# petitioner/MOAI-FHE-TransformerInference-Public

Measured on AMD Instinct MI355X. Metric: NTT+INTT algorithmic GB/s (N=2^16, L=44x60-bit, batch=256 ciphertexts/GPU) vs HBM peak, higher is better.
Workload: dtype u64; 1 GPU; configs[1]: negacyclic NTT then INTT, N=65536, 44 x 60-bit primes, 256 ciphertexts x 2 polys per GPU; batch_per_gpu=256, batch_total=256, coeff_modulus=CoeffModulus::Create(65536, 44 x 60), bytes_per_coeff_per_transform=16

## Files before the change

### moai-fhe-transformerinference-public_amd/csrc/launch.h

```cpp
#pragma once
#include <type_traits>

#include "common.h"
#include "rowlaunch.h"

namespace moai {

#define MOAI_KNOBS(X)                                                                                                          \
    X(NTT_FP, 1, "0: primes below 2^51 stay on the integer units in every transform, key switch and mod-down")                \
    X(NTT_LAZY8, 1, "0: integer primes below 2^60 take the exact butterflies instead of the approximate Shoup quotient")       \
    X(NTT_LAZY16, 1, "0: those primes keep values below 8q with a guard in every stage instead of below 16q with fewer (M_LAZY8)") \
    X(NTT_LDSTW, 1, "0: the forward contiguous pass loads its first stages' twiddles from memory instead of through LDS")      \
    X(NTT_CHUNK_MB, 88, "> 0: launch the two passes of a transform per chunk of whole polynomials of at most this many MiB")    \
    X(NTT_CHUNK_KB, 0, "KiB added to MOAI_NTT_CHUNK_MB: chunks of rings whose polynomials are smaller than a MiB")             \
    X(NTT_PIPE, 2, "1..3: deal those chunks to this many side streams, so that a chunk's second pass runs beside the next one's first; 0: one stream") \
    X(NTT_PIPE_MIN, 32, "chunks per side stream below which a transform stays on the caller's stream")                         \
    X(NTT_PIPE_INNER, 0, "1: the transforms inside key switch, mod-down, encode and decode take the MOAI_NTT_PIPE schedule too") \
    X(NTT_NAIVE, 0, "1: one launch per radix-2 stage over global memory (cross-check path)")                                   \
    X(KS_FP_MIN_ROWS, 16, "batch * L from which the key switch uses the FP64 arithmetic modes")                                \
    X(KS_TMP_MB, 8192, "MiB of key-switch digits in flight: sets how many output moduli share a launch")                       \
    X(KS_P1_ITEMS, 8, "1: the key switch's strided pass at N = 2^16 runs one tile per workgroup instead of eight, pipelined")  \
    X(KS_HOIST_PAIR, 4, "rotations per pass of the hoisted MAC in the FP64 modes: 4, 2, or 0 for one")                         \
    X(MD_FP_MIN_ROWS, 256, "polynomials * L from which mod-down and rescale use the FP64 arithmetic modes")                    \
    X(MATMUL_FP, 1, "0: moai_ct_pt_matmul keeps primes below 2^51 on the integer kernel")                                      \
    X(DEC_TMP_MB, 1024, "MiB of scratch per chunk of moai_ckks_decode when the stream's arena is smaller")                     \
    X(CLIENT_TMP_KB, 1048576, "KiB of scratch per chunk of the encryption and key generation calls when the stream's arena is smaller") \
    X(HYBRID_TMP_KB, 16777216, "KiB of scratch per chunk of the hybrid key switch: sets how many ciphertexts of a batch are in flight") \
    X(HYBRID_HOIST_NR, 4, "rotations per pass of the hybrid hoisted MAC over the digits: 4, 2 or 1")

enum Knob
{
#define MOAI_KNOB_ID(id, dflt, what) K_##id,
    MOAI_KNOBS(MOAI_KNOB_ID)
#undef MOAI_KNOB_ID
    KNOB_COUNT
};
long tuning(Knob k);

template <int... Vs, class F>
int dispatch(const char *what, int v, F &&f)
{
    int rc = MOAI_OK;
    const bool found = ((v == Vs && ((rc = f(std::integral_constant<int, Vs>{})), true)) || ...);
    return found ? rc : set_error(MOAI_ELOGIC, "unsupported %s%d", what, v);
}
template <class F>
int dispatch_logn(int logn, F &&f)
{
    return dispatch<12, 13, 14, 15, 16>("poly_modulus_degree 2^", logn, f);
}
template <class F>
int for_chunks(size_t n, size_t per, F &&f)
{
    for (size_t x0 = 0; x0 < n; x0 += per)
    {
        MOAI_TRY(f(x0, n - x0 < per ? n - x0 : per));
    }
    return MOAI_OK;
}
template <class F>
int for_term_chunks(size_t terms, size_t per, F &&f)
{
    return terms ? for_chunks(terms, per, f) : f(0, 0);
}
inline bool overlap(const void *a, size_t a_bytes, const void *b, size_t b_bytes)
{
    const uintptr_t x = (uintptr_t)a, y = (uintptr_t)b;
    return x < y + b_bytes && y < x + a_bytes;
}
void trace_op(const char *name, size_t L, size_t units);
bool noguard_ok(uint64_t q);
int enter_device(const moai_ctx *c);
int ntt_mode(const moai_ctx *c, uint32_t prime, bool allow_fp = true);
int fwd_class(const moai_ctx *c, uint32_t prime);
int inv_class(const moai_ctx *c, uint32_t prime);
struct TwPair
{
    const Tw *tw, *twb;
};
TwPair twiddles(const moai_ctx *c, int mode, bool inverse);
struct NttArgs;
NttArgs ntt_args(const moai_ctx *c, uint64_t *data, size_t n_poly, size_t L, const RowMap &rows, bool inverse);
int make_rowmap(const moai_ctx *c, size_t L, const uint32_t *prime_index, RowMap *out);
int rows_entry(const moai_ctx *c, size_t L, const uint32_t *prime_index, RowMap *out);
int ntt_launch(moai_ctx *c, uint64_t *data, size_t n_poly, size_t L, const RowMap &rows, bool inverse,
               hipStream_t s, const uint64_t *src = nullptr, size_t src_stride_rows = 0, size_t src_off_rows = 0, bool entry = false);
size_t ntt_pipe_plan(size_t n_poly, size_t L, size_t n, size_t chunk_bytes, long k, long min_chunks, size_t *chunk_polys = nullptr,
                     int *streams = nullptr);
moai_ctx::NttPipe *ntt_pipe(moai_ctx *c, hipStream_t s);
int workspace(moai_ctx *c, size_t bytes, hipStream_t s, void **out);
size_t chunk_items(moai_ctx *c, hipStream_t s, size_t per_bytes, size_t n, size_t cap, size_t floor_bytes);
int reserve_for_stream(moai_ctx *c, void *stream, size_t bytes, void **out, bool headroom);
int galois_table(moai_ctx *c, uint32_t elt, const uint32_t **out);
int galois_permute_c0(moai_ctx *c, const uint64_t *in, uint64_t *out, size_t batch, size_t L, uint32_t galois_elt, hipStream_t s);
int galois_sign_mask(moai_ctx *c, uint64_t *mask, uint32_t galois_elt, size_t copies, hipStream_t s);
int probe_any_zero(moai_ctx *c, const uint64_t *v, size_t words, uint32_t *flag, hipStream_t s, bool *found);
int galois_elt_check(const moai_ctx *c, uint32_t elt);
int moddown_finalize(moai_ctx *c, const uint64_t *acc, uint32_t acc_stride, const uint64_t *u, uint64_t *out, size_t P, size_t Lout,
                     const Tw *inv, const KsAddend &add, const KsList *lst, hipStream_t s);
int galois_gather_list(moai_ctx *c, const KsList *lst, uint64_t *out, size_t members, size_t rows_per_member, size_t src_off_rows,
                       hipStream_t s);
int ks_list_write(const KsList &h, KsList *d, hipStream_t s);
int ks_list_check_members(const uint64_t *const *ins, uint64_t *const *outs, const uint32_t *elts, const uint64_t *const *keys,
                          const uint64_t *one_key, size_t n, bool relin);
int ks_list_check_blocks(const moai_ctx *c, const uint64_t *const *ins, uint64_t *const *outs, const uint32_t *elts,
                         const uint64_t *const *sums, size_t n, size_t in_bytes, size_t out_bytes, bool relin);

int ensure_ckks_tables(moai_ctx *c);
int total_coeff_bits(const moai_ctx *c, size_t L, const uint32_t *prime_index);

size_t rescale_ws_bytes(const moai_ctx *c, size_t L, size_t polys);
int rescale_nolock(moai_ctx *c, const uint64_t *in, uint64_t *out, size_t size, size_t L, size_t batch, hipStream_t s);

int encrypt_zero_key_level(moai_ctx *c, const uint8_t *key, uint64_t seq, const uint64_t *sk_ntt, uint64_t *out, size_t n_batch,
                           hipStream_t s);

int seal_uniform_launch(moai_ctx *c, const uint8_t *seeds, uint64_t *out, size_t stride_words, size_t count, size_t L,
                        const RowMap &rows, uint32_t *cnt, uint32_t *rejected, hipStream_t s);

}
```

### moai-fhe-transformerinference-public_amd/csrc/ntt.hip

```cpp
#include <mutex>

#include "ntt_kernels.hip.h"
#include "launch.h"

namespace moai {

bool noguard_ok(uint64_t q)
{
    return q < (~0ull) / 36;
}

int ntt_mode(const moai_ctx *c, uint32_t prime, bool allow_fp)
{
    const int m = (int)c->pc_host[prime].fp_mode;
    if (allow_fp && m && tuning(K_NTT_FP))
    {
        return m;
    }
    return noguard_ok(c->primes[prime]) ? M_NOGUARD : M_GUARD;
}

TwPair twiddles(const moai_ctx *c, int mode, bool inverse)
{
    if (mode_fp(mode))
    {
        return inverse ? TwPair{ c->inv_twf, c->inv_twfb } : TwPair{ c->fwd_twf, c->fwd_twfb };
    }
    return inverse ? TwPair{ c->inv_tw, c->inv_twb } : TwPair{ c->fwd_tw, c->fwd_twb };
}

static bool lazy8_ok(const moai_ctx *c, uint32_t prime)
{
    return tuning(K_NTT_LAZY8) && c->primes[prime] < (1ull << 60);
}
static bool lazy16_ok(const moai_ctx *c, uint32_t prime)
{
    return lazy8_ok(c, prime) && tuning(K_NTT_LAZY16);
}

int fwd_class(const moai_ctx *c, uint32_t prime)
{
    const int m = ntt_mode(c, prime);
    if (m != M_GUARD)
    {
        return m;
    }
    return lazy16_ok(c, prime) ? M_LAZY16 : (lazy8_ok(c, prime) ? M_LAZY8 : M_GUARD2);
}

int inv_class(const moai_ctx *c, uint32_t prime)
{
    const int m = ntt_mode(c, prime);
    if (mode_fp(m))
    {
        return m;
    }
    return lazy16_ok(c, prime) ? M_LAZY16 : (lazy8_ok(c, prime) ? M_LAZY8 : M_GUARD);
}

NttArgs ntt_args(const moai_ctx *c, uint64_t *data, size_t n_poly, size_t L, const RowMap &rows, bool inverse)
{
    NttArgs a;
    const TwPair t = twiddles(c, M_GUARD, inverse);
    a.data = data;
    a.tw = t.tw;
    a.twb = t.twb;
    a.pc = c->pc;
    a.rows = rows;
    for (size_t r = 0; r < MOAI_MAX_RNS; ++r)
    {
        a.sel.idx[r] = (uint32_t)(r < L ? r : 0);
        a.selp.idx[r] = rows.idx[r < L ? r : 0];
    }
    a.Lsel = (uint32_t)L;
    a.L = (uint32_t)L;
    a.n_poly = (uint32_t)n_poly;
    a.total_work = 0;
    a.src = nullptr;
    a.src_stride = a.src_off = 0;
    a.lds_twiddles = tuning(K_NTT_LDSTW) ? 1u : 0u;
    return a;
}

template <int LOGN, int MODE>
static void launch_fwd_mode(const NttArgs &a, hipStream_t s)
{
    hipLaunchKernelGGL((ntt_fwd_strided<LOGN, MODE>), dim3(a.total_work), dim3(256), 0, s, a);
    if constexpr (MODE == M_LAZY16)
    {
        if (a.lds_twiddles)
        {
            hipLaunchKernelGGL((ntt_fwd_contig<LOGN, MODE, 1>), dim3(a.total_work), dim3(256), 0, s, a);
        }
        else
        {
            hipLaunchKernelGGL((ntt_fwd_contig<LOGN, MODE, 0>), dim3(a.total_work), dim3(256), 0, s, a);
        }
    }
    else
    {
        hipLaunchKernelGGL((ntt_fwd_contig<LOGN, MODE>), dim3(a.total_work), dim3(256), 0, s, a);
    }
}

static void select_class(const moai_ctx *c, int (*row_class)(const moai_ctx *, uint32_t), int mode, NttArgs &a)
{
    a.Lsel = 0;
    for (uint32_t r = 0; r < a.L; ++r)
    {
        const uint32_t prime = a.rows.idx[r];
        if (row_class(c, prime) == mode)
        {
            a.selp.idx[a.Lsel] = prime;
            a.sel.idx[a.Lsel++] = r;
        }
    }
}

template <int LOGN, bool INV, int... MODES>
static int launch_classes(const moai_ctx *c, const NttArgs &base, hipStream_t s)
{
    for (int mode : { MODES... })
    {
        NttArgs a = base;
        select_class(c, INV ? inv_class : fwd_class, mode, a);
        if (a.Lsel == 0)
        {
            continue;
        }
        const TwPair t = twiddles(c, mode, INV);
        a.tw = t.tw;
        a.twb = t.twb;
        a.total_work = a.n_poly * a.Lsel * (1u << (LOGN - 12));
        MOAI_TRY((dispatch<MODES...>(INV ? "inverse transform mode " : "forward transform mode ", mode, [&](auto MD) {
            constexpr int MODE = decltype(MD)::value;
            if constexpr (INV)
            {
                hipLaunchKernelGGL((ntt_inv_contig<LOGN, MODE>), dim3(a.total_work), dim3(256), 0, s, a);
                hipLaunchKernelGGL((ntt_inv_strided<LOGN, MODE>), dim3(a.total_work), dim3(256), 0, s, a);
            }
            else
            {
                launch_fwd_mode<LOGN, MODE>(a, s);
            }
            return MOAI_OK;
        })));
    }
    return MOAI_OK;
}

template <int LOGN>
static int launch_fwd(const moai_ctx *c, const NttArgs &base, hipStream_t s)
{
    return launch_classes<LOGN, false, M_LAZY16, M_LAZY8, M_GUARD2, M_NOGUARD, M_FPN, M_FPR>(c, base, s);
}

template <int LOGN>
static int launch_inv(const moai_ctx *c, const NttArgs &base, hipStream_t s)
{
    return launch_classes<LOGN, true, M_GUARD, M_LAZY8, M_FPN, M_FPR, M_LAZY16>(c, base, s);
}

size_t ntt_pipe_plan(size_t n_poly, size_t L, size_t n, size_t chunk_bytes, long k, long min_chunks, size_t *chunk_polys, int *streams)
{
    size_t chunk = n_poly, per_stream = 0;
    int nk = 0;
    if (n_poly && L && n && chunk_bytes)
    {
        const size_t poly_bytes = L > (~(size_t)0) / sizeof(uint64_t) / n ? ~(size_t)0 : L * n * sizeof(uint64_t);
        chunk = chunk_bytes / poly_bytes;
        chunk = chunk < 1 ? 1 : (chunk > n_poly ? n_poly : chunk);
    }
    const size_t chunks = chunk ? (n_poly + chunk - 1) / chunk : 0;
    if (k >= 1 && chunks >= 2)
    {
        nk = k > NTT_PIPE_MAX ? NTT_PIPE_MAX : (int)k;
        nk = (size_t)nk > chunks ? (int)chunks : nk;
        per_stream = (chunks + (size_t)nk - 1) / (size_t)nk;
        if (min_chunks > 0 && per_stream < (size_t)min_chunks)
        {
            nk = 0;
            per_stream = 0;
        }
    }
    if (chunk_polys)
    {
        *chunk_polys = chunk;
    }
    if (streams)
    {
        *streams = nk;
    }
    return per_stream;
}

int ntt_launch(moai_ctx *c, uint64_t *data, size_t n_poly, size_t L, const RowMap &rows, bool inverse, hipStream_t s,
               const uint64_t *src, size_t src_stride_rows, size_t src_off_rows, bool entry)
{
    if (n_poly == 0 || L == 0)
    {
        return MOAI_OK;
    }
    if (src && !inverse)
    {
        return set_error(MOAI_ELOGIC, "only the inverse transform reads from another buffer");
    }
    if (src && (src_stride_rows > 0xffffffffull || src_off_rows > 0xffffffffull || src_off_rows + L > src_stride_rows))
    {
        return set_error(MOAI_EINVAL, "source slice outside its layout");
    }
    if (n_poly * L * (c->n >> (c->logn >= 12 ? 12 : 0)) > 0x7fffffffull || n_poly > 0xffffffffull)
    {
        return set_error(MOAI_EINVAL, "batch too large for one launch");
    }
    NttArgs a = ntt_args(c, data, n_poly, L, rows, inverse);
    const int logn = c->logn;
    const bool naive = tuning(K_NTT_NAIVE) != 0;
    if (src)
    {
        if (naive || logn <= 11)
        {
            const size_t row_bytes = c->n * sizeof(uint64_t);
            MOAI_HIP_CHECK(hipMemcpy2DAsync(data, L * row_bytes, src + src_off_rows * c->n, src_stride_rows * row_bytes, L * row_bytes, n_poly,
                                            hipMemcpyDeviceToDevice, s));
        }
        else
        {
            a.src = src;
            a.src_stride = (uint32_t)src_stride_rows;
            a.src_off = (uint32_t)src_off_rows;
        }
    }
    if (naive && logn >= 1)
    {
        const dim3 grid = row_grid(c, n_poly * L);
        if (!inverse)
        {
            for (int st = 0; st < logn; ++st)
            {
                hipLaunchKernelGGL(ntt_stage_global<false>, grid, dim3(256), 0, s, a, logn, st, st == logn - 1);
            }
        }
        else
        {
            for (int st = logn - 1; st >= 0; --st)
            {
                hipLaunchKernelGGL(ntt_stage_global<true>, grid, dim3(256), 0, s, a, logn, st, st == 0);
            }
        }
        MOAI_LAUNCH_CHECK();
        return MOAI_OK;
    }
    if (logn <= 11)
    {
        dim3 grid((uint32_t)(n_poly * L));
        if (inverse)
        {
            hipLaunchKernelGGL(ntt_small<true>, grid, dim3(256), 0, s, a, logn);
        }
        else
        {
            hipLaunchKernelGGL(ntt_small<false>, grid, dim3(256), 0, s, a, logn);
        }
        MOAI_LAUNCH_CHECK();
        return MOAI_OK;
    }
    size_t chunk = n_poly;
    int nk = 0;
    const long chunk_mb = tuning(K_NTT_CHUNK_MB), chunk_kb = tuning(K_NTT_CHUNK_KB);
    const size_t chunk_bytes = ((size_t)(chunk_mb > 0 ? chunk_mb : 0) << 20) + ((size_t)(chunk_kb > 0 ? chunk_kb : 0) << 10);
    const long want = tuning(K_NTT_PIPE);
    ntt_pipe_plan(n_poly, L, c->n, chunk_bytes, want > 0 && (entry || tuning(K_NTT_PIPE_INNER)) ? want : 0, tuning(K_NTT_PIPE_MIN), &chunk,
                  &nk);
    moai_ctx::NttPipe *pipe = nullptr;
    if (nk > 0)
    {
        hipStreamCaptureStatus cap = hipStreamCaptureStatusNone;
        if (hipStreamIsCapturing(s, &cap) != hipSuccess)
        {
            (void)hipGetLastError();
        }
        else if (cap == hipStreamCaptureStatusNone)
        {
            pipe = ntt_pipe(c, s);
        }
    }
    std::unique_lock<std::mutex> pipe_lock;
    if (want > 0 && !pipe)
    {
        chunk = n_poly;
    }
    if (pipe)
    {
        pipe_lock = std::unique_lock<std::mutex>(*static_cast<std::mutex *>(pipe->mu));
        MOAI_HIP_CHECK(hipEventRecord(pipe->fork, s));
        for (int i = 0; i < nk; ++i)
// ... 112 lines not shown
```

### moai-fhe-transformerinference-public_amd/csrc/ntt_kernels.hip.h

```cpp
#pragma once
#include "modarith.hip.h"

namespace moai {

__device__ __forceinline__ uint32_t xcd_remap(uint32_t b, uint32_t total)
{
    if (total & 7u)
    {
        return b;
    }
    return (b & 7u) * (total >> 3) + (b >> 3);
}

__device__ __forceinline__ void lds_barrier()
{
    asm volatile("s_waitcnt lgkmcnt(0)\n\ts_barrier" ::: "memory");
}

__device__ __forceinline__ void lds_wave_sync()
{
    asm volatile("s_waitcnt lgkmcnt(0)" ::: "memory");
}

__device__ __forceinline__ uint32_t phys_contig(uint32_t e)
// ... 341 lines not shown
    const uint32_t blk = (tile << 4) + b;
    const Tw *__restrict__ twbt = twb + (size_t)tile * (15 * 256);

    const bool use_lds = TWL < 0 ? ldstw != nullptr : TWL == 1;
    Tw fill;
    uint32_t fill_slot = 0;
    if (use_lds)
    {
        const uint32_t lane = tid & 63u;
        if (TWL == 1)
        {
            const uint32_t l = lane < 59u ? lane : 59u;
            const uint32_t bb = ((tid >> 6) << 2) + l / 15u, i = l % 15u;
            const uint32_t u = i == 0 ? 0u : (i < 3 ? 1u : (i < 7 ? 2u : 3u)), k = i - ((1u << u) - 1u);
            fill = tw[(1u << (R1 + u)) + (((tile << 4) + bb) << u) + k];
            fill_slot = bb * 15u + i;
        }
        else if (lane < 60u)
        {
            const uint32_t bb = ((tid >> 6) << 2) + lane / 15u, i = lane % 15u;
            const uint32_t u = i == 0 ? 0u : (i < 3 ? 1u : (i < 7 ? 2u : 3u)), k = i - ((1u << u) - 1u);
            ldstw[bb * 15u + i] = tw[(1u << (R1 + u)) + (((tile << 4) + bb) << u) + k];
        }
    }
    uint64_t x[16];
#pragma unroll
    for (int j = 0; j < 16; ++j)
    {
        x[j] = base[(b << 8) | ((uint32_t)j << 4) | tl];
    }
    if (use_lds)
    {
        if (TWL == 1 && (tid & 63u) < 60u)
        {
            ldstw[fill_slot] = fill;
        }
        lds_wave_sync();
    }
#pragma unroll
    for (int u = 0; u < 4; ++u)
    {
        const int half = 8 >> u;
#pragma unroll
        for (int j = 0; j < 16; ++j)
        {
            if (!(j & half))
            {
                Tw t = use_lds ? ldstw[b * 15u + ((1u << u) - 1u) + (uint32_t)(j >> (4 - u))]
                               : tw[(1u << (R1 + u)) + (blk << u) + (uint32_t)(j >> (4 - u))];
                ct_bfly_stage<MODE, LOGN>(x[j], x[j + half], t.w, t.wq, q, q2, 7 - u);
            }
        }
    }
#pragma unroll
    for (int j = 0; j < 16; ++j)
    {
        lds[phys_contig((b << 8) | ((uint32_t)j << 4) | tl)] = x[j];
    }
    lds_wave_sync();
    const uint32_t myrow = tid;
#pragma unroll
    for (int c = 0; c < 8; ++c)
    {
        ulonglong2 v = lds2[(myrow << 3) | ((uint32_t)c ^ (myrow & 7u))];
        x[2 * c] = v.x;
        x[2 * c + 1] = v.y;
    }
#pragma unroll
    for (int u = 4; u < 8; ++u)
    {
        const int half = 8 >> (u - 4);
#pragma unroll
        for (int j = 0; j < 16; ++j)
        {
            if (!(j & half))
            {
                Tw t = twbt[(((1u << (u - 4)) - 1u + (uint32_t)(j >> (8 - u))) << 8) + tid];
                ct_bfly_stage<MODE, LOGN>(x[j], x[j + half], t.w, t.wq, q, q2, 7 - u);
            }
        }
    }
#pragma unroll
    for (int c = 0; c < 8; ++c)
    {
        ulonglong2 v;
        if (mode_fp(MODE))
        {
            v.x = fp_to_canonical(u2d(x[2 * c]), u2d(q), u2d(q2));
            v.y = fp_to_canonical(u2d(x[2 * c + 1]), u2d(q), u2d(q2));
        }
        else if (MODE == M_NOGUARD)
        {
            v.x = barrett64(x[2 * c], q, cr1);
            v.y = barrett64(x[2 * c + 1], q, cr1);
        }
        else if (mode_lazy(MODE))
        {
            v.x = lazy_final(x[2 * c], q, cr1);
            v.y = lazy_final(x[2 * c + 1], q, cr1);
        }
        else if (MODE == M_GUARD2)
        {
            v.x = csub(csub(csub(x[2 * c], q2 << 1), q2), q);
            v.y = csub(csub(csub(x[2 * c + 1], q2 << 1), q2), q);
        }
        else
        {
            v.x = csub(csub(x[2 * c], q2), q);
            v.y = csub(csub(x[2 * c + 1], q2), q);
        }
        lds2[(myrow << 3) | ((uint32_t)c ^ (myrow & 7u))] = v;
    }
    lds_wave_sync();
    const uint32_t wbase = (tid >> 6) << 9, lane = tid & 63u;
#pragma unroll
    for (int h = 0; h < 2; ++h)
    {
        uint32_t chs[4];
#pragma unroll
        for (int i = 0; i < 4; ++i)
        {
            chs[i] = wbase + (uint32_t)(4 * h + i) * 64u + lane;
        }
        store.fetch(chs);
#pragma unroll
        for (int i = 0; i < 4; ++i)
        {
            const uint32_t rr = chs[i] >> 3;
            store(i, chs[i], lds2[(rr << 3) | ((chs[i] & 7u) ^ (rr & 7u))]);
        }
    }
}

template <int LOGN, int MODE, int TWL = -1>
__global__ __launch_bounds__(256, 4) void ntt_fwd_contig(NttArgs a)
{
    constexpr uint32_t TPR = 1u << (LOGN - 12);
    __shared__ ulonglong2 lds2[2048 + 240];
    const uint32_t w = xcd_remap(blockIdx.x, a.total_work);
    const uint32_t pol = w % a.n_poly;
    const uint32_t rest = w / a.n_poly;
    const uint32_t tile = rest % TPR;
    const uint32_t r = __builtin_amdgcn_readfirstlane(a.sel.idx[rest / TPR]);
    const uint32_t prime = __builtin_amdgcn_readfirstlane(a.selp.idx[rest / TPR]);
    const PrimeConst &pc = a.pc[prime];
    uint64_t *rowp = a.data + (((size_t)pol * a.L + r) << LOGN);
    StoreTile st;
    st.out = reinterpret_cast<ulonglong2 *>(rowp + ((size_t)tile << 12));
    fwd_contig_tile<LOGN, MODE, StoreTile, TWL>(rowp, tile, a.tw + ((size_t)prime << LOGN), mode_q<MODE>(pc), mode_q2<MODE>(pc), lds2, threadIdx.x,
                                                a.twb + (size_t)prime * ((size_t)TPR * 15 * 256), mode_fin<MODE>(pc), st,
                                                (TWL < 0 ? a.lds_twiddles != 0 : TWL == 1) ? reinterpret_cast<Tw *>(lds2 + 2048) : nullptr);
}

template <int MODE>
__device__ __forceinline__ void gs_bfly_tile(uint64_t (&x)[16], int j, int half, uint64_t w, uint64_t wq, uint64_t q, uint64_t q2, const bool redsum,
                                             uint32_t xk, int i)
{
    if constexpr (MODE == M_LAZY16)
    {
        if (lazy16_inv_kind(xk, i, j, half))
        {
            gs_bfly_lazy16<1>(x[j], x[j + half], w, wq, q, q2);
        }
        else
        {
            gs_bfly_lazy16<0>(x[j], x[j + half], w, wq, q, q2);
        }
    }
    else
    {
        gs_bfly_t<MODE>(x[j], x[j + half], w, wq, q, q2, redsum);
    }
}

template <int LOGN, int MODE>
__device__ __forceinline__ void inv_contig_tile(uint64_t *rowp, uint32_t tile, const Tw *__restrict__ tw,
                                                uint64_t q, uint64_t q2, ulonglong2 *lds2, const uint32_t tid,
                                                const Tw *__restrict__ twb, const uint64_t *srcp = nullptr, Tw *ldstw = nullptr)
{
    static_assert(MODE != M_GUARD2 && MODE != M_NOGUARD, "M_GUARD2 and M_NOGUARD have no inverse butterflies");
    constexpr int R1 = LOGN - 8;
    uint64_t *lds = reinterpret_cast<uint64_t *>(lds2);
    uint64_t *base = rowp + ((size_t)tile << 12);
    const uint32_t b = tid >> 4;
    const uint32_t tl = tid & 15u;
    const uint32_t blk = (tile << 4) + b;
    const Tw *__restrict__ twbt = twb + (size_t)tile * (15 * 256);
    constexpr Lazy16Inv z1 = lazy16_inv(4, 4, false), z2 = lazy16_inv(4, z1.out, false);
    static_assert(z1.peak <= 16 && z2.peak <= 16, "a value of 16q or more");
    static_assert(z2.out == lazy16_inv_handover(), "the strided pass starts from another bound");

    Tw tb[15];
#pragma unroll
    for (int i = 0; i < 15; ++i)
    {
        tb[i] = twbt[((uint32_t)i << 8) + tid];
    }
    if (ldstw)
    {
        const uint32_t ln = tid & 63u;
        if (ln < 60u)
        {
            const uint32_t bb = ((tid >> 6) << 2) + ln / 15u, i = ln % 15u;
            const uint32_t u = i == 0 ? 0u : (i < 3 ? 1u : (i < 7 ? 2u : 3u)), k = i - ((1u << u) - 1u);
            ldstw[bb * 15u + i] = tw[(1u << (R1 + u)) + (((tile << 4) + bb) << u) + k];
        }
    }
    const ulonglong2 *in2 = reinterpret_cast<const ulonglong2 *>(srcp ? srcp + ((size_t)tile << 12) : base);
    const uint32_t wbase = (tid >> 6) << 9, lane = tid & 63u;
#pragma unroll
    for (int it = 0; it < 8; ++it)
    {
        uint32_t ch = wbase + (uint32_t)it * 64u + lane;
        uint32_t rr = ch >> 3;
        lds2[(rr << 3) | ((ch & 7u) ^ (rr & 7u))] = in2[ch];
    }
    lds_wave_sync();
    const uint32_t myrow = tid;
    uint64_t x[16];
#pragma unroll
    for (int c = 0; c < 8; ++c)
    {
        ulonglong2 v = lds2[(myrow << 3) | ((uint32_t)c ^ (myrow & 7u))];
        x[2 * c] = MODE == M_FPN ? d2u(fp_red(fp_from_u52(v.x), u2d(q), u2d(q2))) : (MODE == M_FPR ? d2u(fp_from_u52(v.x)) : v.x);
        x[2 * c + 1] = MODE == M_FPN ? d2u(fp_red(fp_from_u52(v.y), u2d(q), u2d(q2))) : (MODE == M_FPR ? d2u(fp_from_u52(v.y)) : v.y);
    }
#pragma unroll
    for (int u = 7; u >= 4; --u)
    {
        const int half = 8 >> (u - 4);
#pragma unroll
        for (int j = 0; j < 16; ++j)
        {
            if (!(j & half))
            {
                Tw t = tb[(1 << (u - 4)) - 1 + (j >> (8 - u))];
                gs_bfly_tile<MODE>(x, j, half, t.w, t.wq, q, q2, (u & 3) == 0, z1.xk, 7 - u);
            }
        }
    }
#pragma unroll
    for (int c = 0; c < 8; ++c)
    {
        ulonglong2 v;
        v.x = x[2 * c];
        v.y = x[2 * c + 1];
        lds2[(myrow << 3) | ((uint32_t)c ^ (myrow & 7u))] = v;
    }
    lds_wave_sync();
#pragma unroll
    for (int j = 0; j < 16; ++j)
    {
        x[j] = lds[phys_contig((b << 8) | ((uint32_t)j << 4) | tl)];
    }
#pragma unroll
    for (int u = 3; u >= 0; --u)
    {
        const int half = 8 >> u;
#pragma unroll
        for (int j = 0; j < 16; ++j)
        {
            if (!(j & half))
            {
                Tw t = ldstw ? ldstw[b * 15u + ((1u << u) - 1u) + (uint32_t)(j >> (4 - u))]
                             : tw[(1u << (R1 + u)) + (blk << u) + (uint32_t)(j >> (4 - u))];
                gs_bfly_tile<MODE>(x, j, half, t.w, t.wq, q, q2, (u & 3) == 0, z2.xk, 3 - u);
            }
        }
    }
#pragma unroll
    for (int j = 0; j < 16; ++j)
    {
        base[(b << 8) | ((uint32_t)j << 4) | tl] = x[j];
    }
}

template <int LOGN, int MODE>
__global__ __launch_bounds__(256) void ntt_inv_contig(NttArgs a)
{
    constexpr uint32_t TPR = 1u << (LOGN - 12);
    __shared__ ulonglong2 lds2[2048];
    const uint32_t w = xcd_remap(blockIdx.x, a.total_work);
    const uint32_t pol = w % a.n_poly;
    const uint32_t rest = w / a.n_poly;
    const uint32_t tile = rest % TPR;
    const uint32_t r = __builtin_amdgcn_readfirstlane(a.sel.idx[rest / TPR]);
    const uint32_t prime = __builtin_amdgcn_readfirstlane(a.selp.idx[rest / TPR]);
    const PrimeConst &pc = a.pc[prime];
    const uint64_t *srcp = a.src ? a.src + (((size_t)pol * a.src_stride + a.src_off + r) << LOGN) : nullptr;
    inv_contig_tile<LOGN, MODE>(a.data + (((size_t)pol * a.L + r) << LOGN), tile, a.tw + ((size_t)prime << LOGN), mode_q<MODE>(pc),
                                mode_q2<MODE>(pc), lds2, threadIdx.x, a.twb + (size_t)prime * ((size_t)TPR * 15 * 256), srcp);
}

constexpr bool inv_strided_occ4(int mode)
{
    return mode_lazy(mode);
}
template <int LOGN, int MODE>
__device__ __forceinline__ void inv_strided_tile(uint64_t *__restrict__ rowp, uint32_t tile, const Tw *__restrict__ tw,
                                                 const PrimeConst *pc, uint64_t *lds, const uint32_t tid)
{
    static_assert(MODE != M_GUARD2 && MODE != M_NOGUARD, "M_GUARD2 and M_NOGUARD have no inverse butterflies");
    constexpr int R1 = LOGN - 8;
    constexpr int RB = R1 - 4;
    constexpr int GB = 12 - R1;
    constexpr uint32_t G = 1u << GB;
    const uint64_t q = mode_q<MODE>(*pc), q2 = mode_q2<MODE>(*pc);
    uint64_t *__restrict__ row = rowp + tile * G;
    constexpr Lazy16Inv zb = lazy16_inv(RB, lazy16_inv_handover(), false), za = lazy16_inv(4, zb.out, true);
    static_assert(zb.peak <= 16 && za.peak <= 16, "a value of 16q or more");
    static_assert(za.out <= 4 && za.xlast <= 2, "the final subtractions expect products below 4q and the sums times N^-1 below 2q");

    constexpr bool LDSTW = LOGN == 16 && inv_strided_occ4(MODE);
    Tw *ldstw = reinterpret_cast<Tw *>(lds + 4096);
    uint64_t x[16];
    if (RB > 0)
    {
        const uint32_t g = tid & (G - 1);
        const uint32_t th = tid >> GB;
        if (LDSTW)
        {
            ldstw[tid] = tw[tid];
        }
#pragma unroll
        for (int j = 0; j < 16; ++j)
        {
            uint32_t t_ = (th << 4) | (uint32_t)j;
            x[j] = row[(t_ << 8) | g];
        }
        if (LDSTW)
        {
            lds_barrier();
        }
#pragma unroll
        for (int s = R1 - 1; s >= 4; --s)
        {
            const int half = 1 << (R1 - 1 - s);
#pragma unroll
            for (int j = 0; j < 16; ++j)
            {
                if (!(j & half))
                {
                    uint32_t t_ = (th << 4) | (uint32_t)j;
                    Tw t = LDSTW ? ldstw[(1u << s) + (t_ >> (R1 - s))] : tw[(1u << s) + (t_ >> (R1 - s))];
                    gs_bfly_tile<MODE>(x, j, half, t.w, t.wq, q, q2, ((R1 - 1 - s) & 3) == 3, zb.xk, R1 - 1 - s);
                }
            }
        }
#pragma unroll
        for (int j = 0; j < 16; ++j)
        {
            lds[phys_strided<GB>((th << (GB + 4)) | ((uint32_t)j << GB) | g)] = x[j];
        }
        __syncthreads();
#pragma unroll
        for (int j = 0; j < 16; ++j)
        {
            x[j] = lds[phys_strided<GB>((uint32_t)j * 256u + tid)];
        }
    }
    else
    {
#pragma unroll
        for (int j = 0; j < 16; ++j)
        {
            uint32_t e = (uint32_t)j * 256u + tid;
            x[j] = row[((e >> GB) << 8) + (e & (G - 1))];
        }
    }
#pragma unroll
    for (int u = 3; u >= 1; --u)
    {
        const int half = 8 >> u;
#pragma unroll
        for (int j = 0; j < 16; ++j)
        {
            if (!(j & half))
            {
                Tw t = tw[(1u << u) + (uint32_t)(j >> (4 - u))];
                gs_bfly_tile<MODE>(x, j, half, t.w, t.wq, q, q2, ((RB + 3 - u) & 3) == 3, za.xk, 3 - u);
            }
        }
    }
    {
        const Tw ninv = pc->ninv;
        const Tw ninv_w1 = pc->ninv_w1;
        const uint64_t qh = pc->qh;
#pragma unroll
        for (int j = 0; j < 8; ++j)
        {
            if constexpr (MODE == M_LAZY16)
            {
                if (lazy16_inv_kind(za.xk, 3, j, 8))
                {
                    gs_bfly_last_lazy16<1, LOGN>(x[j], x[j + 8], qh, ninv_w1, q, q2);
                }
                else
                {
                    gs_bfly_last_lazy16<0, LOGN>(x[j], x[j + 8], qh, ninv_w1, q, q2);
                }
            }
            else if constexpr (MODE == M_LAZY8)
            {
                gs_bfly_last_lazy8<LOGN>(x[j], x[j + 8], qh, ninv_w1, q, q2);
            }
            else
            {
                gs_bfly_last_t<MODE>(x[j], x[j + 8], ninv, ninv_w1, q, q2);
            }
        }
    }
#pragma unroll
    for (int j = 0; j < 16; ++j)
    {
        uint64_t v;
        if (mode_fp(MODE))
        {
            v = fp_to_canonical(u2d(x[j]), u2d(q), u2d(q2));
        }
        else if (mode_lazy(MODE))
        {
            v = j < 8 ? csub_sign(x[j], q) : csub_sign(csub_sign(x[j], (q2 >> 1) | 0x8000000000000000ull), q);
        }
        else
        {
            v = csub(x[j], q);
        }
        row[((uint32_t)j << (16 - GB)) | ((tid >> GB) << 8) | (tid & (G - 1))] = v;
    }
}

template <int LOGN, int MODE>
__global__ __launch_bounds__(256, inv_strided_occ4(MODE) ? 4 : 5) void ntt_inv_strided(NttArgs a)
{
    constexpr uint32_t TPR = 1u << (LOGN - 12);
    __shared__ uint64_t lds[4096 + ((LOGN == 16 && inv_strided_occ4(MODE)) ? 512 : 0)];
    const uint32_t w = xcd_remap(blockIdx.x, a.total_work);
    const uint32_t tile = w % TPR;
    const uint32_t srow = w / TPR;
    const uint32_t si = srow % a.Lsel;
    const uint32_t r = __builtin_amdgcn_readfirstlane(a.sel.idx[si]);
    const uint32_t prime = __builtin_amdgcn_readfirstlane(a.selp.idx[si]);
    inv_strided_tile<LOGN, MODE>(a.data + ((size_t)((srow / a.Lsel) * a.L + r) << LOGN), tile, a.tw + ((size_t)prime << LOGN), a.pc + prime, lds,
                               threadIdx.x);
// ... 128 lines not shown
```

Measured before the change: 2489 GB/s.

## Pair two polynomials per workgroup in contiguous NTT passes to share twiddles

Adds paired forward and inverse contiguous-pass kernels for the M_LAZY16 mode. Each workgroup processes the same tile of the same prime for two polynomials, so the per-tile twiddle loads are fetched once and reused for both, with a prefetch-ahead queue. The intent is to cut twiddle memory traffic and per-block overhead. The cost is doubled register pressure (two 16-element arrays plus twiddle queues) under launch_bounds(256,4), half as many workgroups, and an extra single-polynomial launch when the count is odd.

```diff
diff --git a/moai-fhe-transformerinference-public_amd/csrc/launch.h b/moai-fhe-transformerinference-public_amd/csrc/launch.h
--- a/moai-fhe-transformerinference-public_amd/csrc/launch.h
+++ b/moai-fhe-transformerinference-public_amd/csrc/launch.h
@@ -11,6 +11,7 @@
     X(NTT_LAZY8, 1, "0: integer primes below 2^60 take the exact butterflies instead of the approximate Shoup quotient")       \
     X(NTT_LAZY16, 1, "0: those primes keep values below 8q with a guard in every stage instead of below 16q with fewer (M_LAZY8)") \
     X(NTT_LDSTW, 1, "0: the forward contiguous pass loads its first stages' twiddles from memory instead of through LDS")      \
+    X(NTT_PAIR, 1, "0: the contiguous passes of the 60-bit rows run one polynomial per workgroup instead of two that share their twiddles") \
     X(NTT_CHUNK_MB, 88, "> 0: launch the two passes of a transform per chunk of whole polynomials of at most this many MiB")    \
     X(NTT_CHUNK_KB, 0, "KiB added to MOAI_NTT_CHUNK_MB: chunks of rings whose polynomials are smaller than a MiB")             \
     X(NTT_PIPE, 2, "1..3: deal those chunks to this many side streams, so that a chunk's second pass runs beside the next one's first; 0: one stream") \
diff --git a/moai-fhe-transformerinference-public_amd/csrc/ntt.hip b/moai-fhe-transformerinference-public_amd/csrc/ntt.hip
--- a/moai-fhe-transformerinference-public_amd/csrc/ntt.hip
+++ b/moai-fhe-transformerinference-public_amd/csrc/ntt.hip
@@ -82,25 +82,72 @@
     return a;
 }
 
+template <int LOGN, int MODE, bool INV>
+static void launch_contig_single(const NttArgs &a, hipStream_t s)
+{
+    if constexpr (INV)
+    {
+        hipLaunchKernelGGL((ntt_inv_contig<LOGN, MODE>), dim3(a.total_work), dim3(256), 0, s, a);
+    }
+    else if constexpr (MODE == M_LAZY16)
+    {
+        if (a.lds_twiddles)
+        {
+            hipLaunchKernelGGL((ntt_fwd_contig<LOGN, MODE, 1>), dim3(a.total_work), dim3(256), 0, s, a);
+        }
+        else
+        {
+            hipLaunchKernelGGL((ntt_fwd_contig<LOGN, MODE, 0>), dim3(a.total_work), dim3(256), 0, s, a);
+        }
+    }
+    else
+    {
+        hipLaunchKernelGGL((ntt_fwd_contig<LOGN, MODE>), dim3(a.total_work), dim3(256), 0, s, a);
+    }
+}
+
+template <int LOGN, int MODE, bool INV>
+static void launch_contig(const NttArgs &a, bool pair, hipStream_t s)
+{
+    if constexpr (contig_pair_mode(MODE))
+    {
+        if (pair && a.n_poly >= 2 && (INV || a.lds_twiddles))
+        {
+            constexpr uint32_t TPR = 1u << (LOGN - 12);
+            NttArgs p = a;
+            p.n_poly = a.n_poly & ~1u;
+            p.total_work = (p.n_poly >> 1) * a.Lsel * TPR;
+            if constexpr (INV)
+            {
+                hipLaunchKernelGGL((ntt_inv_contig2<LOGN, MODE>), dim3(p.total_work), dim3(256), 0, s, p);
+            }
+            else
+            {
+                hipLaunchKernelGGL((ntt_fwd_contig2<LOGN, MODE>), dim3(p.total_work), dim3(256), 0, s, p);
+            }
+            if (a.n_poly & 1u)
+            {
+                NttArgs r = a;
+                r.data = a.data + (((size_t)p.n_poly * a.L) << LOGN);
+                if (a.src)
+                {
+                    r.src = a.src + (((size_t)p.n_poly * a.src_stride) << LOGN);
+                }
+                r.n_poly = 1;
+                r.total_work = a.Lsel * TPR;
+                launch_contig_single<LOGN, MODE, INV>(r, s);
+            }
+            return;
+        }
+    }
+    launch_contig_single<LOGN, MODE, INV>(a, s);
+}
+
 template <int LOGN, int MODE>
-static void launch_fwd_mode(const NttArgs &a, hipStream_t s)
+static void launch_fwd_mode(const NttArgs &a, bool pair, hipStream_t s)
 {
     hipLaunchKernelGGL((ntt_fwd_strided<LOGN, MODE>), dim3(a.total_work), dim3(256), 0, s, a);
-    if constexpr (MODE == M_LAZY16)
-    {
-        if (a.lds_twiddles)
-        {
-            hipLaunchKernelGGL((ntt_fwd_contig<LOGN, MODE, 1>), dim3(a.total_work), dim3(256), 0, s, a);
-        }
-        else
-        {
-            hipLaunchKernelGGL((ntt_fwd_contig<LOGN, MODE, 0>), dim3(a.total_work), dim3(256), 0, s, a);
-        }
-    }
-    else
-    {
-        hipLaunchKernelGGL((ntt_fwd_contig<LOGN, MODE>), dim3(a.total_work), dim3(256), 0, s, a);
-    }
+    launch_contig<LOGN, MODE, false>(a, pair, s);
 }
 
 static void select_class(const moai_ctx *c, int (*row_class)(const moai_ctx *, uint32_t), int mode, NttArgs &a)
@@ -132,16 +179,17 @@
         a.tw = t.tw;
         a.twb = t.twb;
         a.total_work = a.n_poly * a.Lsel * (1u << (LOGN - 12));
+        const bool pair = tuning(K_NTT_PAIR) != 0;
         MOAI_TRY((dispatch<MODES...>(INV ? "inverse transform mode " : "forward transform mode ", mode, [&](auto MD) {
             constexpr int MODE = decltype(MD)::value;
             if constexpr (INV)
             {
-                hipLaunchKernelGGL((ntt_inv_contig<LOGN, MODE>), dim3(a.total_work), dim3(256), 0, s, a);
+                launch_contig<LOGN, MODE, true>(a, pair, s);
                 hipLaunchKernelGGL((ntt_inv_strided<LOGN, MODE>), dim3(a.total_work), dim3(256), 0, s, a);
             }
             else
             {
-                launch_fwd_mode<LOGN, MODE>(a, s);
+                launch_fwd_mode<LOGN, MODE>(a, pair, s);
             }
             return MOAI_OK;
         })));
diff --git a/moai-fhe-transformerinference-public_amd/csrc/ntt_kernels.hip.h b/moai-fhe-transformerinference-public_amd/csrc/ntt_kernels.hip.h
--- a/moai-fhe-transformerinference-public_amd/csrc/ntt_kernels.hip.h
+++ b/moai-fhe-transformerinference-public_amd/csrc/ntt_kernels.hip.h
@@ -517,6 +517,196 @@
                                                 (TWL < 0 ? a.lds_twiddles != 0 : TWL == 1) ? reinterpret_cast<Tw *>(lds2 + 2048) : nullptr);
 }
 
+__device__ __forceinline__ void lds_wave_order()
+{
+    asm volatile("" ::: "memory");
+}
+
+constexpr int PAIR_TW_AHEAD = 8;
+__device__ __forceinline__ void pair_fence(uint64_t &a0, uint64_t &a1, uint64_t &b0, uint64_t &b1)
+{
+    asm volatile("" : "+v"(a0), "+v"(a1), "+v"(b0), "+v"(b1)::"memory");
+}
+constexpr int inv_slot_of_order(int k)
+{
+    return k < 8 ? 7 + k : (k < 12 ? k - 5 : (k < 14 ? k - 11 : 0));
+}
+constexpr int inv_order_of_slot(int s)
+{
+    return s >= 7 ? s - 7 : (s >= 3 ? s + 5 : (s >= 1 ? s + 11 : 14));
+}
+constexpr int slot_stage(int s)
+{
+    return s >= 7 ? 3 : (s >= 3 ? 2 : (s >= 1 ? 1 : 0));
+}
+
+constexpr bool contig_pair_mode(int mode)
+{
+    return mode == M_LAZY16;
+}
+
+template <int LOGN, int MODE>
+__device__ __forceinline__ void fwd_contig_tile2(uint64_t *__restrict__ rowA, uint64_t *__restrict__ rowB, uint32_t tile,
+                                                 const Tw *__restrict__ tw, uint64_t q, uint64_t q2, ulonglong2 *lds2, const uint32_t tid,
+                                                 const Tw *__restrict__ twb, uint64_t cr1, Tw *ldstw)
+{
+    static_assert(contig_pair_mode(MODE) && mode_lazy(MODE), "the paired pass ends in the lazy modes' final reduction");
+    constexpr int R1 = LOGN - 8;
+    uint64_t *lds = reinterpret_cast<uint64_t *>(lds2);
+    uint64_t *__restrict__ baseA = rowA + ((size_t)tile << 12);
+    uint64_t *__restrict__ baseB = rowB + ((size_t)tile << 12);
+    const uint32_t b = tid >> 4;
+    const uint32_t tl = tid & 15u;
+    const Tw *__restrict__ twbt = twb + (size_t)tile * (15 * 256);
+
+    Tw fill;
+    uint32_t fill_slot = 0;
+    {
+        const uint32_t lane = tid & 63u;
+        const uint32_t l = lane < 59u ? lane : 59u;
+        const uint32_t bb = ((tid >> 6) << 2) + l / 15u, i = l % 15u;
+        const uint32_t u = i == 0 ? 0u : (i < 3 ? 1u : (i < 7 ? 2u : 3u)), k = i - ((1u << u) - 1u);
+        fill = tw[(1u << (R1 + u)) + (((tile << 4) + bb) << u) + k];
+        fill_slot = bb * 15u + i;
+    }
+    uint64_t xa[16], xb[16];
+#pragma unroll
+    for (int j = 0; j < 16; ++j)
+    {
+        xa[j] = baseA[(b << 8) | ((uint32_t)j << 4) | tl];
+    }
+#pragma unroll
+    for (int j = 0; j < 16; ++j)
+    {
+        xb[j] = baseB[(b << 8) | ((uint32_t)j << 4) | tl];
+    }
+    if ((tid & 63u) < 60u)
+    {
+        ldstw[fill_slot] = fill;
+    }
+    lds_wave_sync();
+#pragma unroll
+    for (int u = 0; u < 4; ++u)
+    {
+        const int half = 8 >> u;
+#pragma unroll
+        for (int i = 0; i < 8; ++i)
+        {
+            const int j = ((i & ~(half - 1)) << 1) | (i & (half - 1));
+            {
+                Tw t = ldstw[b * 15u + ((1u << u) - 1u) + (uint32_t)(j >> (4 - u))];
+                ct_bfly_stage<MODE, LOGN>(xa[j], xa[j + half], t.w, t.wq, q, q2, 7 - u);
+                ct_bfly_stage<MODE, LOGN>(xb[j], xb[j + half], t.w, t.wq, q, q2, 7 - u);
+            }
+        }
+    }
+    Tw tq[15];
+#pragma unroll
+    for (int s = 0; s < PAIR_TW_AHEAD; ++s)
+    {
+        tq[s] = twbt[((uint32_t)s << 8) + tid];
+    }
+    const uint32_t myrow = tid;
+#pragma unroll
+    for (int j = 0; j < 16; ++j)
+    {
+        lds[phys_contig((b << 8) | ((uint32_t)j << 4) | tl)] = xa[j];
+    }
+    lds_wave_sync();
+#pragma unroll
+    for (int c = 0; c < 8; ++c)
+    {
+        ulonglong2 v = lds2[(myrow << 3) | ((uint32_t)c ^ (myrow & 7u))];
+        xa[2 * c] = v.x;
+        xa[2 * c + 1] = v.y;
+    }
+    lds_wave_order();
+#pragma unroll
+    for (int j = 0; j < 16; ++j)
+    {
+        lds[phys_contig((b << 8) | ((uint32_t)j << 4) | tl)] = xb[j];
+    }
+    lds_wave_sync();
+#pragma unroll
+    for (int c = 0; c < 8; ++c)
+    {
+        ulonglong2 v = lds2[(myrow << 3) | ((uint32_t)c ^ (myrow & 7u))];
+        xb[2 * c] = v.x;
+        xb[2 * c + 1] = v.y;
+    }
+#pragma unroll
+    for (int u = 4; u < 8; ++u)
+    {
+        const int half = 8 >> (u - 4);
+#pragma unroll
+        for (int i = 0; i < 8; ++i)
+        {
+            const int j = ((i & ~(half - 1)) << 1) | (i & (half - 1));
+            {
+                const int slot = (1 << (u - 4)) - 1 + (j >> (8 - u));
+                if ((j & ((1 << (8 - u)) - 1)) == 0)
+                {
+                    if (slot + PAIR_TW_AHEAD < 15)
+                    {
+                        tq[slot + PAIR_TW_AHEAD] = twbt[((uint32_t)(slot + PAIR_TW_AHEAD) << 8) + tid];
+                    }
+                }
+                const Tw t = tq[slot];
+                ct_bfly_stage<MODE, LOGN>(xa[j], xa[j + half], t.w, t.wq, q, q2, 7 - u);
+                ct_bfly_stage<MODE, LOGN>(xb[j], xb[j + half], t.w, t.wq, q, q2, 7 - u);
+                pair_fence(xa[j], xa[j + half], xb[j], xb[j + half]);
+            }
+        }
+    }
+    uint32_t t2 = tid;
+    asm volatile("" : "+v"(t2));
+    const uint32_t wbase = (t2 >> 6) << 9, lane = t2 & 63u;
+#pragma unroll
+    for (int p = 0; p < 2; ++p)
+    {
+        if (p)
+        {
+            lds_wave_order();
+        }
+#pragma unroll
+        for (int c = 0; c < 8; ++c)
+        {
+            ulonglong2 v;
+            v.x = lazy_final(p ? xb[2 * c] : xa[2 * c], q, cr1);
+            v.y = lazy_final(p ? xb[2 * c + 1] : xa[2 * c + 1], q, cr1);
+            lds2[(t2 << 3) | ((uint32_t)c ^ (t2 & 7u))] = v;
+        }
+        lds_wave_sync();
+        ulonglong2 *out = reinterpret_cast<ulonglong2 *>(p ? baseB : baseA);
+#pragma unroll
+        for (int i = 0; i < 8; ++i)
+        {
+            const uint32_t ch = wbase + (uint32_t)i * 64u + lane;
+            const uint32_t rr = ch >> 3;
+            out[ch] = lds2[(rr << 3) | ((ch & 7u) ^ (rr & 7u))];
+        }
+    }
+}
+
+template <int LOGN, int MODE>
+__global__ __launch_bounds__(256, 4) void ntt_fwd_contig2(NttArgs a)
+{
+    constexpr uint32_t TPR = 1u << (LOGN - 12);
+    __shared__ ulonglong2 lds2[2048 + 240];
+    const uint32_t pairs = a.n_poly >> 1;
+    const uint32_t w = xcd_remap(blockIdx.x, a.total_work);
+    const uint32_t pol = (w % pairs) << 1;
+    const uint32_t rest = w / pairs;
+    const uint32_t tile = rest % TPR;
+    const uint32_t r = __builtin_amdgcn_readfirstlane(a.sel.idx[rest / TPR]);
+    const uint32_t prime = __builtin_amdgcn_readfirstlane(a.selp.idx[rest / TPR]);
+    const PrimeConst &pc = a.pc[prime];
+    uint64_t *rowA = a.data + (((size_t)pol * a.L + r) << LOGN);
+    fwd_contig_tile2<LOGN, MODE>(rowA, rowA + ((size_t)a.L << LOGN), tile, a.tw + ((size_t)prime << LOGN), mode_q<MODE>(pc), mode_q2<MODE>(pc),
+                                      lds2, threadIdx.x, a.twb + (size_t)prime * ((size_t)TPR * 15 * 256), mode_fin<MODE>(pc),
+                                      reinterpret_cast<Tw *>(lds2 + 2048));
+}
+
 template <int MODE>
 __device__ __forceinline__ void gs_bfly_tile(uint64_t (&x)[16], int j, int half, uint64_t w, uint64_t wq, uint64_t q, uint64_t q2, const bool redsum,
                                              uint32_t xk, int i)
@@ -655,6 +845,184 @@
     const uint64_t *srcp = a.src ? a.src + (((size_t)pol * a.src_stride + a.src_off + r) << LOGN) : nullptr;
     inv_contig_tile<LOGN, MODE>(a.data + (((size_t)pol * a.L + r) << LOGN), tile, a.tw + ((size_t)prime << LOGN), mode_q<MODE>(pc),
                                 mode_q2<MODE>(pc), lds2, threadIdx.x, a.twb + (size_t)prime * ((size_t)TPR * 15 * 256), srcp);
+}
+
+template <int LOGN, int MODE>
+__device__ __forceinline__ void inv_contig_tile2(uint64_t *rowA, uint64_t *rowB, uint32_t tile, const Tw *__restrict__ tw, uint64_t q,
+                                                 uint64_t q2, ulonglong2 *lds2, const uint32_t tid, const Tw *__restrict__ twb,
+                                                 const uint64_t *srcA, const uint64_t *srcB)
+{
+    static_assert(contig_pair_mode(MODE) && MODE == M_LAZY16, "the paired pass takes M_LAZY16's schedule");
+    constexpr int R1 = LOGN - 8;
+    uint64_t *lds = reinterpret_cast<uint64_t *>(lds2);
+    uint64_t *baseA = rowA + ((size_t)tile << 12);
+    uint64_t *baseB = rowB + ((size_t)tile << 12);
+    const uint32_t b = tid >> 4;
+    const uint32_t tl = tid & 15u;
+    const uint32_t blk = (tile << 4) + b;
+    const Tw *__restrict__ twbt = twb + (size_t)tile * (15 * 256);
+    constexpr Lazy16Inv z1 = lazy16_inv(4, 4, false), z2 = lazy16_inv(4, z1.out, false);
+    static_assert(z1.peak <= 16 && z2.peak <= 16, "a value of 16q or more");
+    static_assert(z2.out == lazy16_inv_handover(), "the strided pass starts from another bound");
+
+    const ulonglong2 *inA = reinterpret_cast<const ulonglong2 *>(srcA ? srcA + ((size_t)tile << 12) : baseA);
+    const ulonglong2 *inB = reinterpret_cast<const ulonglong2 *>(srcB ? srcB + ((size_t)tile << 12) : baseB);
+    const uint32_t wbase = (tid >> 6) << 9, lane = tid & 63u;
+    uint64_t ra[16], rb[16];
+#pragma unroll
+    for (int it = 0; it < 8; ++it)
+    {
+        const ulonglong2 v = inA[wbase + (uint32_t)it * 64u + lane];
+        ra[2 * it] = v.x;
+        ra[2 * it + 1] = v.y;
+    }
+#pragma unroll
+    for (int it = 0; it < 8; ++it)
+    {
+        const ulonglong2 v = inB[wbase + (uint32_t)it * 64u + lane];
+        rb[2 * it] = v.x;
+        rb[2 * it + 1] = v.y;
+    }
+    const uint32_t myrow = tid;
+    uint64_t xa[16], xb[16];
+    auto stage_in = [&](const uint64_t(&raw)[16], uint64_t(&x)[16]) {
+#pragma unroll
+        for (int it = 0; it < 8; ++it)
+        {
+            const uint32_t ch = wbase + (uint32_t)it * 64u + lane;
+            const uint32_t rr = ch >> 3;
+            ulonglong2 v;
+            v.x = raw[2 * it];
+            v.y = raw[2 * it + 1];
+            lds2[(rr << 3) | ((ch & 7u) ^ (rr & 7u))] = v;
+        }
+        lds_wave_sync();
+#pragma unroll
+        for (int c = 0; c < 8; ++c)
+        {
+            ulonglong2 v = lds2[(myrow << 3) | ((uint32_t)c ^ (myrow & 7u))];
+            x[2 * c] = v.x;
+            x[2 * c + 1] = v.y;
+        }
+    };
+    stage_in(ra, xa);
+    Tw tq[15];
+#pragma unroll
+    for (int k = 0; k < PAIR_TW_AHEAD; ++k)
+    {
+        tq[inv_slot_of_order(k)] = twbt[((uint32_t)inv_slot_of_order(k) << 8) + tid];
+    }
+    lds_wave_order();
+    stage_in(rb, xb);
+#pragma unroll
+    for (int u = 7; u >= 4; --u)
+    {
+        const int half = 8 >> (u - 4);
+#pragma unroll
+        for (int i = 0; i < 8; ++i)
+        {
+            const int j = ((i & ~(half - 1)) << 1) | (i & (half - 1));
+            {
+                const int slot = (1 << (u - 4)) - 1 + (j >> (8 - u));
+                if ((j & ((1 << (8 - u)) - 1)) == 0)
+                {
+                    const int k = inv_order_of_slot(slot) + PAIR_TW_AHEAD;
+                    if (k < 15)
+                    {
+                        tq[inv_slot_of_order(k)] = twbt[((uint32_t)inv_slot_of_order(k) << 8) + tid];
+                    }
+                }
+                const Tw t = tq[slot];
+                gs_bfly_tile<MODE>(xa, j, half, t.w, t.wq, q, q2, false, z1.xk, 7 - u);
+                gs_bfly_tile<MODE>(xb, j, half, t.w, t.wq, q, q2, false, z1.xk, 7 - u);
+                pair_fence(xa[j], xa[j + half], xb[j], xb[j + half]);
+            }
+        }
+    }
+    uint32_t t2 = tid;
+    asm volatile("" : "+v"(t2));
+    Tw ts[15];
+#pragma unroll
+    for (int k = 0; k < PAIR_TW_AHEAD; ++k)
+    {
+        const int sl = inv_slot_of_order(k), u = slot_stage(sl);
+        ts[sl] = tw[(1u << (R1 + u)) + (blk << u) + (uint32_t)(sl + 1 - (1 << u))];
+    }
+    auto transpose = [&](uint64_t(&x)[16]) {
+#pragma unroll
+        for (int c = 0; c < 8; ++c)
+        {
+            ulonglong2 v;
+            v.x = x[2 * c];
+            v.y = x[2 * c + 1];
+            lds2[(t2 << 3) | ((uint32_t)c ^ (t2 & 7u))] = v;
+        }
+        lds_wave_sync();
+#pragma unroll
+        for (int j = 0; j < 16; ++j)
+        {
+            x[j] = lds[phys_contig((b << 8) | ((uint32_t)j << 4) | tl)];
+        }
+    };
+    transpose(xa);
+    lds_wave_order();
+    transpose(xb);
+#pragma unroll
+    for (int u = 3; u >= 0; --u)
+    {
+        const int half = 8 >> u;
+#pragma unroll
+        for (int i = 0; i < 8; ++i)
+        {
+            const int j = ((i & ~(half - 1)) << 1) | (i & (half - 1));
+            {
+                const int slot = (1 << u) - 1 + (j >> (4 - u));
+                if ((j & ((1 << (4 - u)) - 1)) == 0)
+                {
+                    const int k = inv_order_of_slot(slot) + PAIR_TW_AHEAD;
+                    if (k < 15)
+                    {
+                        const int sl = inv_slot_of_order(k), un = slot_stage(sl);
+                        ts[sl] = tw[(1u << (R1 + un)) + (blk << un) + (uint32_t)(sl + 1 - (1 << un))];
+                    }
+                }
+                const Tw t = ts[slot];
+                gs_bfly_tile<MODE>(xa, j, half, t.w, t.wq, q, q2, false, z2.xk, 3 - u);
+                gs_bfly_tile<MODE>(xb, j, half, t.w, t.wq, q, q2, false, z2.xk, 3 - u);
+                pair_fence(xa[j], xa[j + half], xb[j], xb[j + half]);
+            }
+        }
+    }
+#pragma unroll
+    for (int j = 0; j < 16; ++j)
+    {
+        baseA[(b << 8) | ((uint32_t)j << 4) | tl] = xa[j];
+    }
+#pragma unroll
+    for (int j = 0; j < 16; ++j)
+    {
+        baseB[(b << 8) | ((uint32_t)j << 4) | tl] = xb[j];
+    }
+}
+
+template <int LOGN, int MODE>
+__global__ __launch_bounds__(256, 4) void ntt_inv_contig2(NttArgs a)
+{
+    constexpr uint32_t TPR = 1u << (LOGN - 12);
+    __shared__ ulonglong2 lds2[2048];
+    const uint32_t pairs = a.n_poly >> 1;
+    const uint32_t w = xcd_remap(blockIdx.x, a.total_work);
+    const uint32_t pol = (w % pairs) << 1;
+    const uint32_t rest = w / pairs;
+    const uint32_t tile = rest % TPR;
+    const uint32_t r = __builtin_amdgcn_readfirstlane(a.sel.idx[rest / TPR]);
+    const uint32_t prime = __builtin_amdgcn_readfirstlane(a.selp.idx[rest / TPR]);
+    const PrimeConst &pc = a.pc[prime];
+    const uint64_t *srcA = a.src ? a.src + (((size_t)pol * a.src_stride + a.src_off + r) << LOGN) : nullptr;
+    uint64_t *rowA = a.data + (((size_t)pol * a.L + r) << LOGN);
+    inv_contig_tile2<LOGN, MODE>(rowA, rowA + ((size_t)a.L << LOGN), tile, a.tw + ((size_t)prime << LOGN), mode_q<MODE>(pc), mode_q2<MODE>(pc), lds2,
+                                 threadIdx.x, a.twb + (size_t)prime * ((size_t)TPR * 15 * 256), srcA,
+                                 srcA ? srcA + ((size_t)a.src_stride << LOGN) : nullptr);
 }
 
 constexpr bool inv_strided_occ4(int mode)
```

New measurement: 2568 GB/s, median of 6. 1.03x the previous value.
